# Ellon/pgslam

Hardware: AMD Instinct MI355X
Metric: ICP-converged scans/sec at 100k-pt scan vs 1M-pt local map (higher is better)
Workload: dtype f32; 1 GPU; scan-to-map ICP, 100000-pt Velodyne-shaped scan vs 1000000-pt local map, <=30 iterations (BASELINE.json configs[1]); distinct_scans=64, matcher=grid, streams=1, parallelism=1 independent replica(s), one process per GPU

## Files before the change

pgslam_amd/csrc/k_launch.inc:

```

static inline int cdiv(long long a, long long b) { return (int)((a + b - 1) / b); }
static inline int round8(int x) { return (x + 7) & ~7; }

template <typename T>
void launch_centroid_bbox_batch(hipStream_t st, const BuildDesc<T> *descs, int n, int max_m, unsigned long long *stats)
{
    int nb = cdiv(max_m, 256 * 8);
    if (nb < 1) nb = 1;
    if (nb > 512) nb = 512;
    hipLaunchKernelGGL(k_centroid_bbox_b<T>, dim3(nb, n), dim3(256), 0, st, descs, stats);
}

template <typename T>
void launch_grid_build_batch(hipStream_t st, const BuildDesc<T> *descs, int n, long long tot_m, long long tot_b, long long tot_s,
                             int max_m, int max_cells, int max_bins, int max_nsc, int max_blocks, int kx_all4, int *fkey, int *bins_a, int *block_sums,
                             int *cell_start, int *cell_start_f, int *bins_b, int *arrival, unsigned long long *words,
                             typename Vec4<T>::type *cpts, typename Vec4<T>::type *cnrm,
                             typename Vec4<T>::type *pts, typename Vec4<T>::type *nrm_out,
                             int *slot_of, int *sc_count, int *near, int *sc_dist, int *sc_wit, unsigned *occ, long long tot_o, float *sc_ext, float *ptsf,
                             uint4 *sw, int *ostart, int *flag_scratch, int *rank_scratch)
{
    (void)hipMemsetAsync(bins_a, 0, sizeof(int) * (tot_b + 1), st);
    (void)hipMemsetAsync(occ, 0, sizeof(unsigned) * tot_o, st);
    (void)hipMemsetAsync(sc_count, 0, sizeof(int) * tot_s, st);
// ... 87 lines not shown
}
constexpr int kTileGroupUnset = -0x7fffffff;
constexpr int kTileGroupDefault = 4;

template <typename T>
void launch_knn(hipStream_t st, int matcher, const ProblemDev *probs, const MapDev<T> *maps, const T *rd, int *slot,
                T *d2, const ChainDev<T> &ch, int P, int max_n, int use_seed, int *slow_count, int2 *slow_list, T *slow_lb,
                int *slow_ring, int fast_rings, const int *active, T *none_r, int n_problems, void *queue_buf, int clear_queue_counters,
                int table_kinds)
{
    if (matcher == 1) {
        (void)hipMemsetAsync(slow_count, 0, 4 * sizeof(int), st);
        hipLaunchKernelGGL(k_knn_brute<T>, dim3(cdiv(max_n, kKnnBlock), P), dim3(kKnnBlock), 0, st, probs, maps, rd, slot, d2,
                           ch, active);
        return;
    }
    const int nseg = n_problems * 8, q_cap = knn_q_cap(max_n);
    char *qb = (char *)queue_buf;
    int *seg_count = (int *)qb;                 qb += sizeof(int) * (size_t)nseg * kQueueCounterStride;
    int *seg_start = (int *)qb;                 qb += (sizeof(int) * (size_t)nseg + 255) & ~(size_t)255;
    int2 *seg_list = (int2 *)qb;                qb += sizeof(int2) * (size_t)nseg * q_cap;
    T *seg_lb = (T *)qb;                        qb += sizeof(T) * (size_t)nseg * q_cap;
    int *seg_ring = (int *)qb;
    if (clear_queue_counters) (void)hipMemsetAsync(seg_count, 0, sizeof(int) * (size_t)nseg * kQueueCounterStride, st);
    {
        static const int forced_lanes = env_knob("PGICP_FAST_LANES", 0);
        int lanes = kFastBlock;
        if ((long long)P * max_n >= 50000)
            while (lanes > 16 && (long long)P * cdiv(max_n, lanes >> 1) <= 8192) lanes >>= 1;
        if (forced_lanes > 0) lanes = std::min(forced_lanes, kFastBlock);
        static const int forced_group = env_knob("PGICP_TILE_GROUP", kTileGroupUnset);
        const int tile_group = forced_group != kTileGroupUnset ? forced_group : kTileGroupDefault;
        if (table_kinds & 1)
            hipLaunchKernelGGL((k_knn_grid<T, 1, 0>), dim3(round8(cdiv(max_n, lanes)), P), dim3(kFastBlock), 0, st, probs, maps, rd, slot, d2, ch,
                               use_seed, fast_rings, seg_count, seg_list, seg_lb, seg_ring, active, none_r, q_cap, lanes, tile_group);
        if (table_kinds & 2)
            hipLaunchKernelGGL((k_knn_grid<T, 1, 1>), dim3(round8(cdiv(max_n, lanes)), P), dim3(kFastBlock), 0, st, probs, maps, rd, slot, d2, ch,
                               use_seed, fast_rings, seg_count, seg_list, seg_lb, seg_ring, active, none_r, q_cap, lanes, tile_group);
    }
    if (P <= 8) {
        hipLaunchKernelGGL(k_queue_small<T>, dim3(P * 8, cdiv(q_cap, 256)), dim3(256), 0, st, (const int *)seg_count, nseg, q_cap,
                           (const int2 *)seg_list, (const T *)seg_lb, (const int *)seg_ring, slow_list, slow_lb, slow_ring, active, slow_count);
        return;
    }
    hipLaunchKernelGGL(k_queue_offsets, dim3(1), dim3(1024), 0, st, (const int *)seg_count, nseg, seg_start, slow_count);
    hipLaunchKernelGGL(k_queue_compact<T>, dim3(P * 8, cdiv(q_cap, 256)), dim3(256), 0, st, (const int *)seg_count, (const int *)seg_start,
                       q_cap, (const int2 *)seg_list, (const T *)seg_lb, (const int *)seg_ring, slow_list, slow_lb, slow_ring, active);
}

template <typename T>
void launch_borrow_order(hipStream_t st, const ProblemDev *probs, const SrcDesc *src, const int *order_a, const int *slot_a, const typename Vec4<T>::type *pts_a,
                         int first_a, int m_a, int n, const SeedSegs &sg, const int *slot_of_b, int m_b, T *rd_sorted, int *order_b, int *slot_b)
{
    hipLaunchKernelGGL(k_borrow_order<T>, dim3(cdiv(n, 256)), dim3(256), 0, st, probs, src, order_a, slot_a, pts_a, first_a, m_a, n, sg, slot_of_b, m_b, rd_sorted, order_b, slot_b);
}

template <typename T>
void launch_knn_med(hipStream_t st, ProblemDev *probs, const MapDev<T> *maps, const T *rd, int *slot, T *d2,
                    const ChainDev<T> &ch, int *slow_count, const int2 *slow_list, T *slow_lb, int *slow_ring, int *slow2_idx,
                    int med_rings, int use_seed, T *none_r)
{
    static const int short_rings = env_knob("PGICP_MED_SHORT_RINGS", 1);
    hipLaunchKernelGGL(k_knn_med<T>, dim3(8192), dim3(64), 0, st, probs, maps, rd, slot, d2, ch, slow_count, slow_list, slow_lb,
                       slow_ring, slow2_idx, med_rings, use_seed, none_r, short_rings);
}

template <typename T>
int launch_knn_topk(hipStream_t st, const ProblemDev *probs, const MapDev<T> *maps, const T *rd, int *slot, T *d2,
                    const ChainDev<T> &ch, int P, int max_n, const int *active)
{
    const dim3 grid(cdiv(max_n, 128), P), block(128);
// ... 337 lines not shown
```

pgslam_amd/csrc/k_match_common.inc:

```

template <typename T>
struct Best {
    T d2;
    int idx;
    int slot;
#ifdef PGICP_KNN_STATS
    int cnt = 0;
#endif
};

#ifdef PGICP_KNN_STATS
__device__ int g_trace_i = -1;
#define KNN_TRACE(prob_, i_, ...) do { if ((prob_) == 0 && (i_) == g_trace_i) printf(__VA_ARGS__); } while (0)
__device__ unsigned long long g_knn_stats[56];
__device__ unsigned *g_cnt_dump = nullptr;
__device__ float *g_d2_dump = nullptr;
__device__ long long g_dump_total = 0;
__device__ int g_dump_passes = 0;
#define KNN_STAT_WAVE_ADD(slot_, v_)                                                              \
    do {                                                                                          \
        long long s_ = (v_);                                                                      \
        for (int o_ = 32; o_ > 0; o_ >>= 1) s_ += __shfl_xor(s_, o_, 64);                          \
        if ((threadIdx.x & 63) == 0) atomicAdd(&g_knn_stats[slot_], (unsigned long long)s_);      \
    } while (0)
#define KNN_STAT_WAVE_MAX(slot_, v_)                                                              \
    do {                                                                                          \
        int s_ = (v_);                                                                            \
        for (int o_ = 32; o_ > 0; o_ >>= 1) s_ = max(s_, __shfl_xor(s_, o_, 64));                  \
        if ((threadIdx.x & 63) == 0) atomicAdd(&g_knn_stats[slot_], (unsigned long long)s_);      \
    } while (0)
#else
#define KNN_TRACE(prob_, i_, ...) do { } while (0)
#endif

#ifdef PGICP_PHASE_STATS
__device__ unsigned long long g_phase[64][3][16];
__device__ unsigned long long g_ball[16];
__device__ unsigned long long g_slow_worst[16];
#define PHASE_BEGIN() long long ph_t = (long long)__builtin_amdgcn_s_memtime(); unsigned ph_d[8] = {0, 0, 0, 0, 0, 0, 0, 0}
#define PHASE_MARK(k_) do { const long long t_ = (long long)__builtin_amdgcn_s_memtime(); ph_d[k_] += (unsigned)(t_ - ph_t); ph_t = t_; } while (0)
#define PHASE_FLUSH() do {                                                                                                  \
        if ((int)(threadIdx.x & 63) == __ffsll((long long)__ballot(1)) - 1) {                                              \
            unsigned long long *dst_ = g_phase[blockIdx.x & 63][use_seed ? 1 : 0];                                          \
            for (int k_ = 0; k_ < 8; ++k_) atomicAdd(dst_ + k_, (unsigned long long)ph_d[k_]);                              \
            atomicAdd(dst_ + 15, 1ULL);                                                                                     \
        } } while (0)
#define SPH_BEGIN() long long sph_t = (long long)__builtin_amdgcn_s_memtime(); const long long sph_t0 = sph_t; long long sph_e0 = sph_t; unsigned sph_emax = 0; unsigned sph_d[8] = {0, 0, 0, 0, 0, 0, 0, 0}; unsigned sph_n = 0
#define SPH_MARK(k_) do { const long long t_ = (long long)__builtin_amdgcn_s_memtime(); sph_d[k_] += (unsigned)(t_ - sph_t); sph_t = t_; } while (0)
#define SPH_ARRIVED(cond_) do { if (cond_) printf("x"); } while (0)
#define SPH_FLUSH() do {                                                                                                    \
        if ((threadIdx.x & 63) == 0) {                                                                                      \
            unsigned long long *dst_ = g_phase[blockIdx.x & 63][2];                                                         \
            for (int k_ = 0; k_ < 8; ++k_) atomicAdd(dst_ + k_, (unsigned long long)sph_d[k_]);                              \
            atomicAdd(dst_ + 14, (unsigned long long)sph_n); atomicAdd(dst_ + 15, 1ULL);                                    \
            atomicMax(dst_ + 12, (unsigned long long)(sph_t - sph_t0)); atomicMax(dst_ + 13, (unsigned long long)sph_emax);  \
        } } while (0)
#else
#define PHASE_BEGIN() do { } while (0)
#define PHASE_MARK(k_) do { } while (0)
#define PHASE_FLUSH() do { } while (0)
#define SPH_BEGIN() do { } while (0)
#define SPH_ARRIVED(cond_) do { } while (0)
#define SPH_MARK(k_) do { } while (0)
#define SPH_FLUSH() do { } while (0)
#endif

#ifdef PGICP_XCC_STATS
constexpr int kXccCopies = 32;
__device__ unsigned long long g_xcc[8][kXccCopies][16];
#define XCC_BEGIN() const unsigned long long xc_t0 = wall_clock64()
// ... 222 lines not shown
```

pgslam_amd/csrc/k_match_fast.inc:

```

template <typename T>
__device__ __forceinline__ T slab_far(T u, T lo, T hi)
{
    return fmax(fabs(u - lo), fabs(hi - u));
}

template <typename T>
__device__ __forceinline__ void finish_query(const MapDev<T> &M, const GridDesc<T> &g, const ChainDev<T> &ch, bool resolved, T gr,
                                             Best<T> best, T qx, T qy, T qz, T ux, T uy, T uz, int cx, int cy, int cz, int prob,
                                             int i, long long pos, int r_next, T lb_override, T free_r, int *__restrict__ slot_io,
                                             T *__restrict__ d2_out, T *__restrict__ none_r,
                                             int *__restrict__ slow_count, int2 *__restrict__ slow_list, T *__restrict__ slow_lb,
                                             int *__restrict__ slow_ring, int q_cap)
{
    if (resolved) {
        if (best.slot < 0) { best.d2 = Bits<T>::inf(); none_r[pos] = fmax(free_r, (T)0); }
        else none_r[pos] = sqrt(best.d2) * (T)0.9999;
    } else {
        T lb = lb_override >= (T)0 ? lb_override : (gr > (T)0 ? gr * gr : (T)0);
        if (free_r > (T)0) lb = fmax(lb, free_r * free_r);
        none_r[pos] = fmax(sqrt(lb) * (T)0.9999, free_r);
        if (best.slot < 0) {
            const int Cx = cx >> 3, Cy = cy >> 3, Cz = cz >> 3;
            const int wslot = as_global(M.sc_wit)[Cx + M.nsx * (Cy + M.nsy * Cz)];
// ... 45 lines not shown

template <typename T>
__global__ __launch_bounds__(256) void k_borrow_order(const ProblemDev *__restrict__ probs, const SrcDesc *__restrict__ src, const int *__restrict__ order_a,
                                                       const int *__restrict__ slot_a, const typename Vec4<T>::type *__restrict__ pts_a, int first_a, int m_a, int n, SeedSegs sg,
                                                       const int *__restrict__ slot_of_b, int m_b, T *__restrict__ rd_sorted, int *__restrict__ order_b,
                                                       int *__restrict__ slot_b)
{
    const int j = blockIdx.x * 256 + threadIdx.x;
    if (j >= n) return;
    const ProblemDev &P = probs[0];
    const SrcDesc sd = src[0];
    const int i = order_a[j];
    const T *in = (const T *)sd.ptr + (long long)i * sd.stride;
    T qx, qy, qz;
    apply_T<T>(P.Tpre, in[0], in[1], in[2], qx, qy, qz);
    T *dst = rd_sorted + 3 * (P.off + j);
    dst[0] = qx; dst[1] = qy; dst[2] = qz;
    order_b[P.off + j] = i;
    const int s = slot_a[j];
    int out = -1;
    if ((unsigned)s - (unsigned)first_a < (unsigned)m_a) {
        const int ia = Bits<T>::unpack_idx(pts_a[s].w);
        for (int k = 0; k < sg.n; ++k)
            if (ia >= sg.src[k] && ia < sg.src[k + 1]) {
                const unsigned off = (unsigned)ia - (unsigned)sg.src[k];
                if (sg.dst[k] >= 0 && sg.dst[k] < m_b && off < (unsigned)(m_b - sg.dst[k])) out = slot_of_b[sg.dst[k] + (int)off];
                break;
            }
    }
    slot_b[P.off + j] = out;
}
constexpr int kFastBlock = PGICP_FAST_BLOCK;

template <typename T, int R, int TK>
__global__ __launch_bounds__(kFastBlock) PGICP_FAST_ATTR void k_knn_grid(const ProblemDev *__restrict__ probs, const MapDev<T> *__restrict__ maps,
                                                  const T *__restrict__ rd, int *__restrict__ slot_io,
                                                  T *__restrict__ d2_out, ChainDev<T> ch, int use_seed, int fast_rings,
                                                  int *__restrict__ slow_count, int2 *__restrict__ slow_list,
                                                  T *__restrict__ slow_lb, int *__restrict__ slow_ring,
                                                  const int *__restrict__ active, T *__restrict__ none_r, int q_cap, int lanes, int tile_group)
{
    using V4 = typename Vec4<T>::type;
    constexpr int NR = (2 * R + 1) * (2 * R + 1);
    constexpr bool kItems = kFastBlock == 64;
    constexpr bool kBallPool = kItems && PGICP_RING_POOL;
    __shared__ __attribute__((aligned(16))) int lds_raw[2 * kItemsMax + (sizeof(T) == 4 ? 6 : 12) * kFastBlock];
    static_assert(sizeof(lds_raw) >= sizeof(int) * 2 * (NR - 1) * kFastBlock && kItemsMax >= (NR - 1) * kFastBlock, "the list view and one item per range must fit");
    int (*rng_a)[kFastBlock] = reinterpret_cast<int (*)[kFastBlock]>(lds_raw);
    int (*rng_b)[kFastBlock] = reinterpret_cast<int (*)[kFastBlock]>(lds_raw + (NR - 1) * kFastBlock);
    const int prob = active[blockIdx.y];
    const ProblemDev &P = probs[prob];
    if (P.done) return;
    const int tile = tile_of_block(blockIdx.x, gridDim.x, tile_group);
    const int lane = threadIdx.x;
    const int i = tile * lanes + lane;
    if (tile * lanes >= P.n) return;
    PHASE_BEGIN();
    XCC_BEGIN();
    bool live = lane < lanes && i < P.n;
    const MapDev<T> M = maps[P.map];
    if ((M.sw != nullptr) != (TK == 1)) return;
    const GridDesc<T> g = M.g;
    T qx = 0, qy = 0, qz = 0;
    const T cap2 = (use_seed & 1) ? (T)(1.21 * P.rlimit) : Bits<T>::inf();
    const bool capped = cap2 < ch.max_dist2;
    bool still_none = false, skip = false;
    T free_r = (T)0;
    Best<T> best, seed;
    best.d2 = capped ? cap2 : ch.max_dist2;
    best.idx = 0x7FFFFFFF;
    best.slot = -1;
    seed.d2 = Bits<T>::inf(); seed.idx = 0x7FFFFFFF; seed.slot = -1;
    int dsc = 0;
    if (live) {
        const T *q = rd + 3 * (P.off + i);
        apply_T<T>(tcur_of<T>(P), q[0], q[1], q[2], qx, qy, qz);
        {
            const int sx = clamp_cell<T>(qx - g.ox, g.inv_h, g.nx) >> 3, sy8 = clamp_cell<T>(qy - g.oy, g.inv_h, g.ny) >> 3,
                      sz8 = clamp_cell<T>(qz - g.oz, g.inv_h, g.nz) >> 3;
// ... 149 lines not shown
#pragma unroll
            for (int u = 0; u < NP; ++u) { c0[u] = load_rec<T>(M.pts, pv[u] ? pj[u] : 0); c1[u] = load_rec<T>(M.pts, pt[u] ? pj[u] + 1 : 0); }
#pragma unroll
            for (int u = 0; u < NP; ++u) {
                eval_point_if<T>(pv[u], c0[u], pj[u], qx, qy, qz, best);
                eval_point_if<T>(pt[u], c1[u], pj[u] + 1, qx, qy, qz, best);
            }
#ifdef PGICP_KNN_STATS
            flat_iters += 2;
#endif
        }
    }
    }
    }
#ifdef PGICP_KNN_STATS
    KNN_STAT_WAVE_MAX(3, flat_iters);
    KNN_STAT_WAVE_ADD(4, best.cnt - cnt_a1);
    if (live) {
        atomicAdd(&g_knn_stats[16 + (cnt_a1 <= 0 ? 0 : min(15, 32 - __clz(cnt_a1)))], 1ULL);
        const int c2 = best.cnt - cnt_a1;
        atomicAdd(&g_knn_stats[32 + (c2 <= 0 ? 0 : min(15, 32 - __clz(c2)))], 1ULL);
    }
    const int cnt_a = best.cnt;
    const bool dump_on = g_cnt_dump && P.iters < g_dump_passes && lane < lanes && i < P.n;
    if (dump_on) {
        g_cnt_dump[(long long)P.iters * g_dump_total + P.off + i] = (unsigned)min(cnt_a1, 1023) | ((unsigned)min(cnt_a - cnt_a1, 1023) << 10);
        g_d2_dump[(long long)P.iters * g_dump_total + P.off + i] = use_seed ? (float)seed.d2 : -1.0f;
    }
#endif
    PHASE_MARK(4);
    if (!__any(live)) { PHASE_FLUSH(); XCC_END(); }
    if constexpr (!kBallPool) { if (!live) return; }

    T gr;
    int r_next;
    bool resolved;
    if constexpr (kBallPool) {
        if constexpr (sizeof(T) == 4)
            resolved = grid_nn_ball<T, TK>(M, lane, search, qx, qy, qz, ch.max_dist, R, fast_rings, cap2, best, gr, r_next, items, sq, skey, nullptr, sslot, pool_n);
        else {
            T *sqd = reinterpret_cast<T *>(lds_raw + 2 * kItemsMax);
            unsigned long long *skd = reinterpret_cast<unsigned long long *>(lds_raw + 2 * kItemsMax + 6 * kFastBlock);
            int *sxd = lds_raw + 2 * kItemsMax + 8 * kFastBlock, *ssd = lds_raw + 2 * kItemsMax + 9 * kFastBlock;
            unsigned *fbd = reinterpret_cast<unsigned *>(lds_raw + 2 * kItemsMax + 10 * kFastBlock);
            float *sud = reinterpret_cast<float *>(lds_raw + 2 * kItemsMax + 11 * kFastBlock);
            resolved = grid_nn_ball<T, TK>(M, lane, search, qx, qy, qz, ch.max_dist, R, fast_rings, cap2, best, gr, r_next, items, sqd, skd, sxd, ssd, pool_n, fbd, sud);
        }
        if (!live) return;
    } else {
        resolved = false; gr = (T)0; r_next = R + 1;
        if (search) resolved = grid_nn<T>(M, qx, qy, qz, ch.max_dist, R + 1, fast_rings, cap2, best, gr, r_next);
    }
    PHASE_MARK(5);
#ifdef PGICP_KNN_STATS
    atomicAdd(&g_knn_stats[5], (unsigned long long)(best.cnt - cnt_a));
    atomicAdd(&g_knn_stats[6], (unsigned long long)(resolved ? 0 : 1));
    atomicAdd(&g_knn_stats[7], (unsigned long long)(best.cnt > cnt_a ? 1 : 0));
    KNN_STAT_WAVE_MAX(8, best.cnt - cnt_a);
    KNN_STAT_WAVE_MAX(9, best.cnt);
    if (dump_on) g_cnt_dump[(long long)P.iters * g_dump_total + P.off + i] |= (unsigned)min(best.cnt - cnt_a, 4095) << 20;
#endif
    KNN_TRACE(prob, i, "[fast] i=%d use_seed=%d capped=%d cap2=%g best=(%g,%d) seed=(%g,%d) resolved=%d gr=%g r_next=%d\n", i, use_seed, (int)capped, (double)cap2, (double)best.d2, best.slot, (double)seed.d2, seed.slot, (int)resolved, (double)gr, r_next);
    T lb_override = (T)-1;
    if (skip) {
        resolved = false;
        r_next = 0;
        gr = (T)0;
    }
    if (capped && best.slot < 0) {
        if (resolved) lb_override = cap2;
        resolved = false;
        if (seed.slot >= 0 && seed.d2 <= ch.max_dist2) best = seed;
// ... 9 lines not shown
```

pgslam_amd/csrc/k_match_pool.inc:

```
#ifndef PGICP_ITEMS_MAX
#define PGICP_ITEMS_MAX 512
#endif
#ifndef PGICP_ITEM_CHUNK
#define PGICP_ITEM_CHUNK 8
#endif
constexpr int kItemsMax = PGICP_ITEMS_MAX;
#ifndef PGICP_ITEM_CHUNK_F
#define PGICP_ITEM_CHUNK_F 4
#endif
#ifndef PGICP_ITEM_CHUNK_D
#define PGICP_ITEM_CHUNK_D PGICP_ITEM_CHUNK
#endif
template <typename T> struct ItemChunk { static constexpr int n = sizeof(T) == 4 ? PGICP_ITEM_CHUNK_F : PGICP_ITEM_CHUNK_D;
                                         static constexpr int shift = n == 4 ? 2 : n == 8 ? 3 : n == 16 ? 4 : n == 32 ? 5 : -1; };
constexpr int kItemShift = ItemChunk<float>::shift;
static_assert(ItemChunk<float>::shift > 0 && ItemChunk<double>::shift > 0, "the item size is a power of two (items are counted with shifts: a division by a run-time size costs ~30 VALU instructions)");

__device__ __forceinline__ void item_rounds(const float4 *__restrict__ pts, const int2 *items, int total, const float *sq,
                                            unsigned long long *skey, int *sslot, int lane, int chunk)
{
    __syncthreads();
    for (int b0 = 0; b0 < total; b0 += 64) {
        const int it = b0 + lane;
        const int2 I = it < total ? items[it] : make_int2(0, 0);
// ... 226 lines not shown
    }
    if (total == 0) return;
    const int chunk = 1 << sh;
    int w = incl - mine;
#pragma unroll
    for (int t = 0; t < N; ++t) {
        const int len = rb[t] - ra[t];
        if (len > 0) { items[w] = make_int2(ra[t], (min(len, chunk) << 6) | lane); ++w; }
        if (__any(len > chunk)) {
#pragma clang loop vectorize(disable) unroll(disable)
            for (int a = ra[t] + chunk; a < rb[t]; a += chunk) { items[w] = make_int2(a, (min(rb[t] - a, chunk) << 6) | lane); ++w; }
        }
    }
    const unsigned long long key0 = (unsigned long long)__double_as_longlong(best.d2);
    const int idx0 = best.idx;
    sq[lane] = qx; sq[64 + lane] = qy; sq[128 + lane] = qz;
    skey[lane] = key0;
    sidx[lane] = idx0;
    sslot[lane] = best.slot;
    if (ptsf) { fb[lane] = __float_as_uint(bk_up(best.d2)); item_rounds_dp(pts, ptsf, items, total, sq, skey, sidx, sslot, fb, su, lane, chunk); }
    else item_rounds_d(pts, items, total, sq, skey, sidx, sslot, lane, chunk);
    const unsigned long long kf = skey[lane];
    const int xf = sidx[lane];
    if (kf != key0 || xf != idx0) { best.d2 = __longlong_as_double((long long)kf); best.idx = xf; best.slot = sslot[lane]; }
}

#ifndef PGICP_RING_POOL
#define PGICP_RING_POOL 1
#endif
#ifndef PGICP_FREE_SKIP
#define PGICP_FREE_SKIP 1
#endif
constexpr int kPoolCap = kItemsMax - 1;
#ifndef PGICP_BALL_ROWS
#define PGICP_BALL_ROWS 2
#endif
constexpr int kBallRows = PGICP_BALL_ROWS;
constexpr int kPoolFlushAt = kPoolCap - 128 * kBallRows;
template <typename T, int TK = 2>
__device__ __forceinline__ bool grid_nn_ball(const MapDev<T> &M, int lane, bool active, T qx, T qy, T qz, T max_dist,
                                             int r_done, int max_rings, T stop_d2, Best<T> &best, T &gr_out, int &r_next,
                                             int2 *items, T *sq, unsigned long long *skey, int *sidx, int *sslot, int *pool_n,
                                             unsigned *fb = nullptr, const float *su = nullptr)
{
    r_next = r_done + 1;
    const GridDesc<T> g = M.g;
    const int c0x = clamp_cell<T>(qx - g.ox, g.inv_h, g.nx), c0y = clamp_cell<T>(qy - g.oy, g.inv_h, g.ny), c0z = clamp_cell<T>(qz - g.oz, g.inv_h, g.nz);
    GridDesc<BK> gb;
    gb.h = (BK)g.h; gb.inv_h = (BK)g.inv_h; gb.margin = bk_margin<T>(g, qx - g.ox, qy - g.oy, qz - g.oz); gb.nx = g.nx; gb.ny = g.ny; gb.nz = g.nz;
    const BK ux = (BK)(qx - g.ox), uy = (BK)(qy - g.oy), uz = (BK)(qz - g.oz);
    const BK bmax = (BK)max_dist, bstop = (BK)stop_d2;
    BK bbest = bk_up(best.d2);
    gr_out = (T)0;
    bool resolved = false, open = active;
    if (open) {
        BK gr = ring_guarantee<BK>(gb, ux, uy, uz, c0x, c0y, c0z, r_done);
        if (!(gr < Bits<BK>::inf())) { resolved = true; open = false; }
        else {
            gr = gr - gb.margin;
            gr_out = (T)gr;
            if (gr > (BK)0 && (bbest < gr * gr || gr > bmax)) { resolved = true; open = false; }
            else if (gr > (BK)0 && gr * gr > bstop) open = false;
        }
    }
    if (max_rings <= r_done || !__any(open)) return resolved;
    const typename Vec4<T>::type *pts = M.pts;
    const int kx = M.kx, nxf = g.nx * kx;
    const BK inv_hx = gb.inv_h * (BK)kx;
    const int sy = __builtin_amdgcn_readfirstlane(nxf), sz = __builtin_amdgcn_readfirstlane(nxf * g.ny);
    sq[lane] = qx; sq[64 + lane] = qy; sq[128 + lane] = qz;
    if constexpr (sizeof(T) == 4) skey[lane] = item_key(best.d2, best.idx);
    else { skey[lane] = (unsigned long long)__double_as_longlong(best.d2); sidx[lane] = best.idx; if (fb) fb[lane] = __float_as_uint(bk_up(best.d2)); }
    sslot[lane] = best.slot;
    if (lane == 0) *pool_n = 0;
    __syncthreads();
#ifdef PGICP_PHASE_STATS
    int st_trips = 0, st_items = 0, st_flush = 0;
#endif
    auto push = [&](int a, int b) {
        constexpr int kItemChunk = ItemChunk<T>::n;
        const int n = (b - a + kItemChunk - 1) >> ItemChunk<T>::shift;
        const int w = atomicAdd(pool_n, n);
        if (w + n <= kPoolCap) {
            items[w] = make_int2(a, (min(b - a, kItemChunk) << 6) | lane);
#pragma clang loop vectorize(disable) unroll(disable)
            for (int k = 1; k < n; ++k) items[w + k] = make_int2(a + k * kItemChunk, (min(b - a - k * kItemChunk, kItemChunk) << 6) | lane);
        } else {
#pragma clang loop vectorize(disable) unroll(disable)
            for (int k = w; k < kPoolCap; ++k) items[k] = make_int2(0, lane);
            scan_range<T>(pts, a, b, qx, qy, qz, best);
        }
    };
    auto flush = [&]() {
        __syncthreads();
        const int total = min(__builtin_amdgcn_readfirstlane(*pool_n), kPoolCap);
        if (total > 0) {
#ifdef PGICP_PHASE_STATS
            st_items += total; ++st_flush;
#endif
            if constexpr (sizeof(T) == 4) {
                item_rounds(pts, items, total, sq, skey, sslot, lane, ItemChunk<T>::n);
                const unsigned long long kf = skey[lane];
                if (kf < item_key(best.d2, best.idx)) { best.d2 = __uint_as_float((unsigned)(kf >> 32)); best.idx = (int)(unsigned)kf; best.slot = sslot[lane]; }
            } else {
                if (fb && M.ptsf) item_rounds_dp(pts, reinterpret_cast<const float4 *>(M.ptsf), items, total, sq, skey, sidx, sslot, fb, su, lane, ItemChunk<T>::n);
                else item_rounds_d(pts, items, total, sq, skey, sidx, sslot, lane, ItemChunk<T>::n);
                const unsigned long long kf = skey[lane], kb = (unsigned long long)__double_as_longlong(best.d2);
                const int xf = sidx[lane];
                if (kf < kb || (kf == kb && xf < best.idx)) { best.d2 = __longlong_as_double((long long)kf); best.idx = xf; best.slot = sslot[lane]; }
                skey[lane] = (unsigned long long)__double_as_longlong(best.d2); sidx[lane] = best.idx; sslot[lane] = best.slot;
                if (fb) fb[lane] = __float_as_uint(bk_up(best.d2));
            }
            bbest = bk_up(best.d2);
            if (lane == 0) *pool_n = 0;
            __syncthreads();
        }
    };
    const BK rho = bk_sqrt(bbest) * (BK)1.000001 + gb.margin;
    const int ylo = max(c0y - max_rings, clamp_cell<BK>(uy - rho, gb.inv_h, g.ny)), yhi = min(c0y + max_rings, clamp_cell<BK>(uy + rho, gb.inv_h, g.ny));
    const int zlo = max(c0z - max_rings, clamp_cell<BK>(uz - rho, gb.inv_h, g.nz)), zhi = min(c0z + max_rings, clamp_cell<BK>(uz + rho, gb.inv_h, g.nz));
    const BK wl_all = (BK)(max(c0x - max_rings, 0) * kx), wh_all = (BK)(min(c0x + max_rings, g.nx - 1) * kx + kx - 1);
    const BK wh_left = (BK)((c0x - r_done) * kx - 1), wl_right = (BK)((c0x + r_done) * kx + kx);
#ifdef PGICP_PHASE_STATS
    const int st_open = __popcll(__ballot(open));
    int st_rows = open ? (yhi - ylo + 1) * (zhi - zlo + 1) : 0;
    for (int o_ = 32; o_ > 0; o_ >>= 1) st_rows += __shfl_xor(st_rows, o_, 64);
#endif
    int y = ylo, z = zlo;
    int rowb = nxf * (ylo + g.ny * zlo);
    const int wrap = sz - (yhi - ylo + 1) * sy;
    bool walking = open;
#if PGICP_BALL_ROWS > 1
    while (__any(walking)) {
        constexpr int NW = 2 * kBallRows;
        int ia[NW], ib[NW];
        bool need[NW];
#pragma unroll
        for (int w = 0; w < NW; ++w) { ia[w] = 0; ib[w] = 0; need[w] = false; }
#pragma unroll
        for (int r = 0; r < kBallRows; ++r) {
            if (walking) {
                const BK ly = fmax(slab_dist<BK>(uy, y, gb.h) - gb.margin, (BK)0), lz = fmax(slab_dist<BK>(uz, z, gb.h) - gb.margin, (BK)0);
                const BK lb2 = ly * ly + lz * lz;
                if (!(lb2 > bbest)) {
                    const BK rad = bk_sqrt(fmax(bbest - lb2, (BK)0)) * (BK)1.000001 + gb.margin;
                    const BK flo = floor((ux - rad) * inv_hx), fhi = floor((ux + rad) * inv_hx);
                    const bool inside = abs(y - c0y) <= r_done && abs(z - c0z) <= r_done;
#pragma unroll
                    for (int k = 0; k < 2; ++k) {
                        const BK wl = (inside && k == 1) ? wl_right : wl_all, wh = (inside && k == 0) ? wh_left : wh_all;
                        const bool on = (k == 0 || inside) && !(wl > wh || fhi < wl || flo > wh);
                        need[2 * r + k] = on;
                        ia[2 * r + k] = rowb + (int)fmax(flo, wl); ib[2 * r + k] = rowb + (int)fmin(fhi, wh) + 1;
                    }
                }
                ++y; rowb += sy;
                if (y > yhi) { y = ylo; ++z; rowb += wrap; walking = z <= zhi; }
            }
        }
        int va[NW], vb[NW];
#pragma unroll
        for (int w = 0; w < NW; ++w) { va[w] = 0; vb[w] = 0; if (need[w]) tab_range_k<TK, T>(M, ia[w], ib[w], va[w], vb[w]); }
#pragma unroll
        for (int w = 0; w < NW; ++w) if (va[w] < vb[w]) push(va[w], vb[w]);
#ifdef PGICP_PHASE_STATS
        ++st_trips;
#endif
        __syncthreads();
        if (__builtin_amdgcn_readfirstlane(*pool_n) >= kPoolFlushAt) flush();
    }
#else
    while (__any(walking)) {
        if (walking) {
            const BK ly = fmax(slab_dist<BK>(uy, y, gb.h) - gb.margin, (BK)0), lz = fmax(slab_dist<BK>(uz, z, gb.h) - gb.margin, (BK)0);
            const BK lb2 = ly * ly + lz * lz;
            if (!(lb2 > bbest)) {
                const BK rad = bk_sqrt(fmax(bbest - lb2, (BK)0)) * (BK)1.000001 + gb.margin;
                const BK flo = floor((ux - rad) * inv_hx), fhi = floor((ux + rad) * inv_hx);
                const bool inside = abs(y - c0y) <= r_done && abs(z - c0z) <= r_done;
#pragma unroll 1
                for (int k = 0; k < (inside ? 2 : 1); ++k) {
                    const BK wl = (inside && k == 1) ? wl_right : wl_all, wh = (inside && k == 0) ? wh_left : wh_all;
                    if (wl > wh || fhi < wl || flo > wh) continue;
                    const int fa = (int)fmax(flo, wl), fb = (int)fmin(fhi, wh);
                    int a, b;
                    tab_range_k<TK, T>(M, rowb + fa, rowb + fb + 1, a, b);
                    if (a < b) push(a, b);
                }
            }
            ++y; rowb += sy;
            if (y > yhi) { y = ylo; ++z; rowb += wrap; walking = z <= zhi; }
        }
#ifdef PGICP_PHASE_STATS
        ++st_trips;
#endif
        __syncthreads();
        if (__builtin_amdgcn_readfirstlane(*pool_n) >= kPoolFlushAt) flush();
    }
#endif
    flush();
#ifdef PGICP_PHASE_STATS
    if (lane == 0) {
        atomicAdd(&g_ball[0], 1ULL); atomicAdd(&g_ball[1], (unsigned long long)st_open); atomicAdd(&g_ball[2], (unsigned long long)st_trips);
        atomicAdd(&g_ball[4], (unsigned long long)st_items); atomicAdd(&g_ball[5], (unsigned long long)st_flush);
        atomicAdd(&g_ball[7], (unsigned long long)st_rows);
    }
#endif
    if (open) {
        BK gr = ring_guarantee<BK>(gb, ux, uy, uz, c0x, c0y, c0z, max_rings);
        if (!(gr < Bits<BK>::inf())) resolved = true;
        else {
            gr = gr - gb.margin;
            gr_out = (T)gr;
            bbest = bk_up(best.d2);
            if (gr > (BK)0 && (bbest < gr * gr || gr > bmax)) resolved = true;
            else r_next = max_rings + 1;
        }
    }
    return resolved;
}
```

pgslam_amd/csrc/k_minimise.inc:

```

__device__ __forceinline__ void accumulate_pair(double *acc, double w, double px, double py, double pz, double qx,
                                                double qy, double qz, double nx, double ny, double nz)
{
    const double dx = px - qx, dy = py - qy, dz = pz - qz;
    const double e = (nx * dx + ny * dy) + nz * dz;
    double J[6];
    J[0] = py * nz - pz * ny;
    J[1] = pz * nx - px * nz;
    J[2] = px * ny - py * nx;
    J[3] = nx; J[4] = ny; J[5] = nz;
    int k = 0;
#pragma unroll
    for (int a = 0; a < 6; a++)
#pragma unroll
        for (int b = a; b < 6; b++) acc[k++] += w * (J[a] * J[b]);
#pragma unroll
    for (int a = 0; a < 6; a++) acc[21 + a] -= w * (J[a] * e);
    acc[27] += w;
    acc[28] += 1.0;
    acc[29] += w * (e * e);
}

constexpr int kDppShl4 = 0x104, kDppShr4 = 0x114, kDppRor8 = 0x128, kDppQuadXor2 = 0x4E, kDppQuadXor1 = 0xB1;

// ... 438 lines not shown

__global__ __launch_bounds__(256) void k_reopen(ProblemDev *__restrict__ probs, int P)
{
    const int p = blockIdx.x * blockDim.x + threadIdx.x;
    if (p < P && probs[p].status == PGICP_ST_OK) probs[p].done = 0;
}
void launch_reopen(hipStream_t st, ProblemDev *probs, int P)
{
    hipLaunchKernelGGL(k_reopen, dim3((P + 255) / 256), dim3(256), 0, st, probs, P);
}

int knn_trace_set(int sorted_index)
{
#ifdef PGICP_KNN_STATS
    return hipMemcpyToSymbol(HIP_SYMBOL(g_trace_i), &sorted_index, sizeof(int)) == hipSuccess ? 0 : -1;
#else
    (void)sorted_index;
    return -1;
#endif
}

int knn_phase_read(unsigned long long out[48], int reset)
{
#ifdef PGICP_PHASE_STATS
    static unsigned long long h[64 * 48];
    if (hipMemcpyFromSymbol(h, HIP_SYMBOL(g_phase), sizeof h) != hipSuccess) return -1;
    for (int k = 0; k < 48; k++) {
        out[k] = 0;
        const bool is_max = k == 32 + 12 || k == 32 + 13;
        for (int c = 0; c < 64; c++) out[k] = is_max ? std::max(out[k], h[c * 48 + k]) : out[k] + h[c * 48 + k];
    }
    if (reset) { std::memset(h, 0, sizeof h); (void)hipMemcpyToSymbol(HIP_SYMBOL(g_phase), h, sizeof h); }
    {
        unsigned long long b[16];
        if (hipMemcpyFromSymbol(b, HIP_SYMBOL(g_ball), sizeof b) == hipSuccess && b[0])
            std::fprintf(stderr, "      ball walk: %llu waves; per wave: %.1f open lanes, %.1f trips, %.1f items in %.2f evaluations; %.1f rows per open lane\n",
                         b[0], (double)b[1] / b[0], (double)b[2] / b[0], (double)b[4] / b[0], (double)b[5] / b[0], b[1] ? (double)b[7] / b[1] : 0.0);
        if (reset) { std::memset(b, 0, sizeof b); (void)hipMemcpyToSymbol(HIP_SYMBOL(g_ball), b, sizeof b); }
    }
    {
        unsigned long long w[16];
        if (hipMemcpyFromSymbol(w, HIP_SYMBOL(g_slow_worst), sizeof w) == hipSuccess && w[0])
            std::fprintf(stderr, "      slowest entry: %llu cycles [fetch %llu seed %llu look-ups %llu points %llu walk %llu finish %llu]; square of %llu rows, %llu with points, %llu long, %llu candidates; bounded %llu capped %llu, result at %llu mm\n",
                         w[0], w[1], w[2], w[3], w[4], w[5], w[6], w[8], w[9], w[10], w[11], w[12], w[13], w[14]);
        if (reset) { std::memset(w, 0, sizeof w); (void)hipMemcpyToSymbol(HIP_SYMBOL(g_slow_worst), w, sizeof w); }
    }
    return 0;
#else
    (void)out; (void)reset;
    return -1;
#endif
}

int knn_xcc_report(int use_seed, int reset)
{
#ifdef PGICP_XCC_STATS
    static unsigned long long h[8][kXccCopies][16];
    if (hipMemcpyFromSymbol(h, HIP_SYMBOL(g_xcc), sizeof h) != hipSuccess) return -1;
    unsigned long long x[8][16] = {};
    for (int c = 0; c < 8; c++)
        for (int k = 0; k < kXccCopies; k++)
            for (int s = 0; s < 16; s++) x[c][s] = s < 2 ? std::max(x[c][s], h[c][k][s]) : x[c][s] + h[c][k][s];
    unsigned long long first = ~0ULL;
    for (int c = 0; c < 8; c++) if (x[c][3]) first = std::min(first, ~x[c][0]);
    std::fprintf(stderr, "    fast kernel per XCC (seeded %d) [last end after the launch's first start | wave time summed | waves | waves by blockIdx.x & 7], ticks of 10 ns:", use_seed);
    for (int c = 0; c < 8; c++) {
        std::fprintf(stderr, " %llu|%llu|%llu|", x[c][3] ? x[c][1] - first : 0ULL, x[c][2], x[c][3]);
        for (int k = 0; k < 8; k++) std::fprintf(stderr, "%s%llu", k ? "," : "", x[c][8 + k]);
    }
    std::fprintf(stderr, "\n");
// ... 288 lines not shown
```

pgslam_amd/csrc/kernels.hip:

```cpp
#include "kernels.hpp"
#include "tile_map.hpp"
#include <algorithm>
#include <cstdio>
#include <cstdlib>
#include <cstring>
#include <limits>
#include <map>
#include <type_traits>
#ifndef PGICP_FAST_BLOCK
#define PGICP_FAST_BLOCK 64
#endif
#ifndef PGICP_FAST_WAVES
#define PGICP_FAST_WAVES 6
#endif
#ifndef PGICP_FAST_ATTR
#ifndef PGICP_FAST_WAVES_D
#define PGICP_FAST_WAVES_D 4
#endif
#define PGICP_FAST_ATTR __attribute__((amdgpu_num_sgpr(80), amdgpu_waves_per_eu(sizeof(T) == 4 ? PGICP_FAST_WAVES : PGICP_FAST_WAVES_D, sizeof(T) == 4 ? PGICP_FAST_WAVES : PGICP_FAST_WAVES_D)))
#endif

namespace pgicp {

template <typename T> struct Bits;
template <> struct Bits<float> {
    using U = unsigned int;
    static constexpr int kBits = 32;
    __device__ static U key(float v) { return __float_as_uint(v); }
    __device__ static float val(U k) { return __uint_as_float(k); }
    __device__ static float pack_idx(int i) { return __int_as_float(i); }
    __device__ static int unpack_idx(float w) { return __float_as_int(w); }
    __device__ static float inf() { return __uint_as_float(0x7F800000u); }
};
template <> struct Bits<double> {
// ... 138 lines not shown
```

Baseline: 13030 scans/s.

## Deal ball-walk row chunks across wave lanes to balance imbalanced per-lane boxes

Adds a load-balanced mode to the grid ball search. When per-lane row counts are skewed enough, the rows of every lane's yz box are dealt evenly across all 64 lanes through LDS, so each lane scans another lane's rows and pushes items tagged with the owner. It also adds a template flag so the kNN kernel skips the ring-walk path when fast_rings is 1. The dealt mode adds LDS space, extra barriers and per-owner reads from shared memory in exchange for fewer idle lanes in imbalanced waves.

New measurement: 13200 scans/s, median of 6. 1.01x the previous value.

```diff
diff --git a/pgslam_amd/csrc/ball_rows.hpp b/pgslam_amd/csrc/ball_rows.hpp
--- /dev/null
+++ b/pgslam_amd/csrc/ball_rows.hpp
@@ -0,0 +1,35 @@
+#pragma once
+
+#if defined(__HIPCC__) || defined(__CUDACC__)
+#define PGICP_BALL_HD __host__ __device__ __forceinline__
+#else
+#define PGICP_BALL_HD inline
+#endif
+
+namespace pgicp {
+
+constexpr int kBallDealMaxRings = 7;
+
+PGICP_BALL_HD unsigned ball_box_pack(int ny, int nz, int dylo, int dzlo)
+{
+    return ((unsigned)ny << 12) | ((unsigned)nz << 8) | ((unsigned)dylo << 4) | (unsigned)dzlo;
+}
+PGICP_BALL_HD int ball_box_ny(unsigned w) { return (int)((w >> 12) & 15u); }
+PGICP_BALL_HD int ball_box_nz(unsigned w) { return (int)((w >> 8) & 15u); }
+PGICP_BALL_HD int ball_box_dylo(unsigned w) { return (int)((w >> 4) & 15u); }
+PGICP_BALL_HD int ball_box_dzlo(unsigned w) { return (int)(w & 15u); }
+
+PGICP_BALL_HD int ball_chunks(int n, int per) { return (n + per - 1) / per; }
+
+PGICP_BALL_HD void ball_row_yz(int r, int ny, float inv_ny, int &dy, int &dz)
+{
+    dz = (int)(((float)r + 0.5f) * inv_ny);
+    dy = r - dz * ny;
+}
+
+PGICP_BALL_HD int ball_deal_place(int first, int below, int window) { return first - window + below; }
+PGICP_BALL_HD unsigned ball_deal_word(int k, int lane) { return ((unsigned)k << 6) | (unsigned)lane; }
+PGICP_BALL_HD int ball_deal_owner(unsigned w) { return (int)(w & 63u); }
+PGICP_BALL_HD int ball_deal_chunk(unsigned w) { return (int)(w >> 6); }
+
+}
diff --git a/pgslam_amd/csrc/k_launch.inc b/pgslam_amd/csrc/k_launch.inc
--- a/pgslam_amd/csrc/k_launch.inc
+++ b/pgslam_amd/csrc/k_launch.inc
@@ -143,11 +143,11 @@
         static const int forced_group = env_knob("PGICP_TILE_GROUP", kTileGroupUnset);
         const int tile_group = forced_group != kTileGroupUnset ? forced_group : kTileGroupDefault;
         if (table_kinds & 1)
-            hipLaunchKernelGGL((k_knn_grid<T, 1, 0>), dim3(round8(cdiv(max_n, lanes)), P), dim3(kFastBlock), 0, st, probs, maps, rd, slot, d2, ch,
-                               use_seed, fast_rings, seg_count, seg_list, seg_lb, seg_ring, active, none_r, q_cap, lanes, tile_group);
+            hipLaunchKernelGGL((fast_rings > 1 ? k_knn_grid<T, 1, 0, true> : k_knn_grid<T, 1, 0, false>), dim3(round8(cdiv(max_n, lanes)), P), dim3(kFastBlock), 0, st,
+                               probs, maps, rd, slot, d2, ch, use_seed, fast_rings, seg_count, seg_list, seg_lb, seg_ring, active, none_r, q_cap, lanes, tile_group);
         if (table_kinds & 2)
-            hipLaunchKernelGGL((k_knn_grid<T, 1, 1>), dim3(round8(cdiv(max_n, lanes)), P), dim3(kFastBlock), 0, st, probs, maps, rd, slot, d2, ch,
-                               use_seed, fast_rings, seg_count, seg_list, seg_lb, seg_ring, active, none_r, q_cap, lanes, tile_group);
+            hipLaunchKernelGGL((fast_rings > 1 ? k_knn_grid<T, 1, 1, true> : k_knn_grid<T, 1, 1, false>), dim3(round8(cdiv(max_n, lanes)), P), dim3(kFastBlock), 0, st,
+                               probs, maps, rd, slot, d2, ch, use_seed, fast_rings, seg_count, seg_list, seg_lb, seg_ring, active, none_r, q_cap, lanes, tile_group);
     }
     if (P <= 8) {
         hipLaunchKernelGGL(k_queue_small<T>, dim3(P * 8, cdiv(q_cap, 256)), dim3(256), 0, st, (const int *)seg_count, nseg, q_cap,
diff --git a/pgslam_amd/csrc/k_match_common.inc b/pgslam_amd/csrc/k_match_common.inc
--- a/pgslam_amd/csrc/k_match_common.inc
+++ b/pgslam_amd/csrc/k_match_common.inc
@@ -35,7 +35,7 @@
 
 #ifdef PGICP_PHASE_STATS
 __device__ unsigned long long g_phase[64][3][16];
-__device__ unsigned long long g_ball[16];
+__device__ unsigned long long g_ball[2][16];
 __device__ unsigned long long g_slow_worst[16];
 #define PHASE_BEGIN() long long ph_t = (long long)__builtin_amdgcn_s_memtime(); unsigned ph_d[8] = {0, 0, 0, 0, 0, 0, 0, 0}
 #define PHASE_MARK(k_) do { const long long t_ = (long long)__builtin_amdgcn_s_memtime(); ph_d[k_] += (unsigned)(t_ - ph_t); ph_t = t_; } while (0)
diff --git a/pgslam_amd/csrc/k_match_fast.inc b/pgslam_amd/csrc/k_match_fast.inc
--- a/pgslam_amd/csrc/k_match_fast.inc
+++ b/pgslam_amd/csrc/k_match_fast.inc
@@ -101,7 +101,7 @@
 }
 constexpr int kFastBlock = PGICP_FAST_BLOCK;
 
-template <typename T, int R, int TK>
+template <typename T, int R, int TK, bool WALK = true>
 __global__ __launch_bounds__(kFastBlock) PGICP_FAST_ATTR void k_knn_grid(const ProblemDev *__restrict__ probs, const MapDev<T> *__restrict__ maps,
                                                   const T *__restrict__ rd, int *__restrict__ slot_io,
                                                   T *__restrict__ d2_out, ChainDev<T> ch, int use_seed, int fast_rings,
@@ -113,7 +113,7 @@
     constexpr int NR = (2 * R + 1) * (2 * R + 1);
     constexpr bool kItems = kFastBlock == 64;
     constexpr bool kBallPool = kItems && PGICP_RING_POOL;
-    __shared__ __attribute__((aligned(16))) int lds_raw[2 * kItemsMax + (sizeof(T) == 4 ? 6 : 12) * kFastBlock];
+    __shared__ __attribute__((aligned(16))) int lds_raw[2 * kItemsMax + (sizeof(T) == 4 ? 6 + 3 * PGICP_BALL_DEAL : 12) * kFastBlock];
     static_assert(sizeof(lds_raw) >= sizeof(int) * 2 * (NR - 1) * kFastBlock && kItemsMax >= (NR - 1) * kFastBlock, "the list view and one item per range must fit");
     int (*rng_a)[kFastBlock] = reinterpret_cast<int (*)[kFastBlock]>(lds_raw);
     int (*rng_b)[kFastBlock] = reinterpret_cast<int (*)[kFastBlock]>(lds_raw + (NR - 1) * kFastBlock);
@@ -329,12 +329,14 @@
     if (!__any(live)) { PHASE_FLUSH(); XCC_END(); }
     if constexpr (!kBallPool) { if (!live) return; }
 
+    if constexpr (!WALK) fast_rings = R;
     T gr;
     int r_next;
     bool resolved;
     if constexpr (kBallPool) {
         if constexpr (sizeof(T) == 4)
-            resolved = grid_nn_ball<T, TK>(M, lane, search, qx, qy, qz, ch.max_dist, R, fast_rings, cap2, best, gr, r_next, items, sq, skey, nullptr, sslot, pool_n);
+            resolved = grid_nn_ball<T, TK>(M, lane, search, qx, qy, qz, ch.max_dist, R, fast_rings, cap2, best, gr, r_next, items, sq, skey, nullptr, sslot, pool_n, nullptr, nullptr,
+                                            reinterpret_cast<unsigned *>(lds_raw + 2 * kItemsMax + 6 * kFastBlock));
         else {
             T *sqd = reinterpret_cast<T *>(lds_raw + 2 * kItemsMax);
             unsigned long long *skd = reinterpret_cast<unsigned long long *>(lds_raw + 2 * kItemsMax + 6 * kFastBlock);
diff --git a/pgslam_amd/csrc/k_match_pool.inc b/pgslam_amd/csrc/k_match_pool.inc
--- a/pgslam_amd/csrc/k_match_pool.inc
+++ b/pgslam_amd/csrc/k_match_pool.inc
@@ -282,6 +282,12 @@
 #define PGICP_FREE_SKIP 1
 #endif
 constexpr int kPoolCap = kItemsMax - 1;
+#ifndef PGICP_BALL_DEAL
+#define PGICP_BALL_DEAL 1
+#endif
+#ifndef PGICP_BALL_DEAL_GAIN
+#define PGICP_BALL_DEAL_GAIN 65
+#endif
 #ifndef PGICP_BALL_ROWS
 #define PGICP_BALL_ROWS 2
 #endif
@@ -291,7 +297,7 @@
 __device__ __forceinline__ bool grid_nn_ball(const MapDev<T> &M, int lane, bool active, T qx, T qy, T qz, T max_dist,
                                              int r_done, int max_rings, T stop_d2, Best<T> &best, T &gr_out, int &r_next,
                                              int2 *items, T *sq, unsigned long long *skey, int *sidx, int *sslot, int *pool_n,
-                                             unsigned *fb = nullptr, const float *su = nullptr)
+                                             unsigned *fb = nullptr, const float *su = nullptr, [[maybe_unused]] unsigned *sown = nullptr)
 {
     r_next = r_done + 1;
     const GridDesc<T> g = M.g;
@@ -325,7 +331,7 @@
     if (lane == 0) *pool_n = 0;
     __syncthreads();
 #ifdef PGICP_PHASE_STATS
-    int st_trips = 0, st_items = 0, st_flush = 0;
+    int st_trips = 0, st_items = 0, st_flush = 0, st_kept = 0;
 #endif
     auto push = [&](int a, int b) {
         constexpr int kItemChunk = ItemChunk<T>::n;
@@ -380,6 +386,135 @@
     int rowb = nxf * (ylo + g.ny * zlo);
     const int wrap = sz - (yhi - ylo + 1) * sy;
     bool walking = open;
+#if PGICP_BALL_DEAL
+    if constexpr (sizeof(T) == 4) {
+        if (max_rings <= kBallDealMaxRings) {
+            const int nyb = yhi - ylo + 1, nzb = zhi - zlo + 1;
+            const int mine = open ? ball_chunks(nyb * nzb, kBallRows) : 0;
+            int total = mine, most = mine;
+#pragma unroll
+            for (int o = 32; o > 0; o >>= 1) { total += __shfl_xor(total, o, 64); most = max(most, __shfl_xor(most, o, 64)); }
+            if (100 * ((total + 63) >> 6) <= PGICP_BALL_DEAL_GAIN * most) {
+                walking = false;
+                unsigned *sfc = sown + 64;
+                sown[lane] = open ? ball_box_pack(nyb, nzb, c0y - ylo, c0z - zlo) : 0u;
+                sfc[lane] = (unsigned)(c0x * kx);
+                unsigned *shead = sown + 128;
+                int lev = 0, lev0 = 0;
+                __syncthreads();
+                const unsigned *skey_hi = reinterpret_cast<const unsigned *>(skey) + 1;
+                auto flush_dealt = [&]() {
+                    __syncthreads();
+                    const int n_items = min(__builtin_amdgcn_readfirstlane(*pool_n), kPoolCap);
+                    if (n_items > 0) {
+#ifdef PGICP_PHASE_STATS
+                        st_items += n_items; ++st_flush;
+#endif
+                        item_rounds(pts, items, n_items, sq, skey, sslot, lane, ItemChunk<T>::n);
+                        if (lane == 0) *pool_n = 0;
+                        __syncthreads();
+                    }
+                };
+                for (int cb = 0; cb < total; cb += 64) {
+                    const bool valid = cb + lane < total;
+                    for (int k = lev, first = lev0; first < cb + 64 && k < most; ++k) {
+                        const unsigned long long in = __ballot(mine > k);
+                        const int pos = ball_deal_place(first, (int)__builtin_amdgcn_mbcnt_hi((unsigned)(in >> 32), __builtin_amdgcn_mbcnt_lo((unsigned)in, 0u)), cb);
+                        if (mine > k && pos >= 0 && pos < 64) shead[pos] = ball_deal_word(k, lane);
+                        first += __popcll(in);
+                        if (first <= cb + 64) { lev = k + 1; lev0 = first; }
+                    }
+                    __syncthreads();
+                    const unsigned hv = shead[lane];
+                    const int owner = ball_deal_owner(hv), lchunk = valid ? ball_deal_chunk(hv) : 0x7FFF;
+                    const unsigned bw = sown[owner];
+                    const int ony = ball_box_ny(bw), orows = ony * ball_box_nz(bw);
+                    const BK oux = sq[owner] - g.ox, ouy = sq[64 + owner] - g.oy, ouz = sq[128 + owner] - g.oz;
+                    const int ocy = clamp_cell<T>(ouy, g.inv_h, g.ny), ocz = clamp_cell<T>(ouz, g.inv_h, g.nz);
+                    const int fc = (int)sfc[owner];
+                    const BK owl_all = (BK)max(fc - max_rings * kx, 0), owh_all = (BK)min(fc + max_rings * kx + kx - 1, nxf - 1);
+                    const BK owh_left = (BK)(fc - r_done * kx - 1), owl_right = (BK)(fc + r_done * kx + kx);
+                    int r = lchunk * kBallRows, dy, dz;
+                    ball_row_yz(r, ony, __builtin_amdgcn_rcpf((float)ony), dy, dz);
+                    const int oylo = ocy - ball_box_dylo(bw);
+                    int yy = oylo + dy, zz = ocz - ball_box_dzlo(bw) + dz;
+                    int orow = nxf * (yy + g.ny * zz);
+                    bool going = valid && r < orows;
+                    const BK obest = __uint_as_float(skey_hi[2 * owner]);
+                    constexpr int NW = 2 * kBallRows;
+                    int ia[NW], ib[NW];
+                    bool need[NW];
+#pragma unroll
+                    for (int w = 0; w < NW; ++w) { ia[w] = 0; ib[w] = 0; need[w] = false; }
+#pragma unroll
+                    for (int k = 0; k < kBallRows; ++k) {
+                        if (going) {
+                            const BK ly = fmax(slab_dist<BK>(ouy, yy, gb.h) - gb.margin, (BK)0), lz = fmax(slab_dist<BK>(ouz, zz, gb.h) - gb.margin, (BK)0);
+                            const BK lb2 = ly * ly + lz * lz;
+                            if (!(lb2 > obest)) {
+#ifdef PGICP_PHASE_STATS
+                                ++st_kept;
+#endif
+                                const BK rad = bk_sqrt(fmax(obest - lb2, (BK)0)) * (BK)1.000001 + gb.margin;
+                                const BK flo = floor((oux - rad) * inv_hx), fhi = floor((oux + rad) * inv_hx);
+                                const bool inside = abs(yy - ocy) <= r_done && abs(zz - ocz) <= r_done;
+#pragma unroll
+                                for (int e = 0; e < 2; ++e) {
+                                    const BK wl = (inside && e == 1) ? owl_right : owl_all, wh = (inside && e == 0) ? owh_left : owh_all;
+                                    const bool on = (e == 0 || inside) && !(wl > wh || fhi < wl || flo > wh);
+                                    need[2 * k + e] = on;
+                                    ia[2 * k + e] = orow + (int)fmax(flo, wl); ib[2 * k + e] = orow + (int)fmin(fhi, wh) + 1;
+                                }
+                            }
+                            ++yy; orow += sy; ++r;
+                            if (yy >= oylo + ony) { yy = oylo; ++zz; orow += sz - ony * sy; }
+                            going = r < orows;
+                        }
+                    }
+                    int va[NW], vb[NW];
+#pragma unroll
+                    for (int w = 0; w < NW; ++w) { va[w] = 0; vb[w] = 0; if (need[w]) tab_range_k<TK, T>(M, ia[w], ib[w], va[w], vb[w]); }
+                    Best<T> ov;
+                    ov.d2 = Bits<T>::inf(); ov.idx = 0x7FFFFFFF; ov.slot = -1;
+#pragma unroll
+                    for (int w = 0; w < NW; ++w) if (va[w] < vb[w]) {
+                        constexpr int kItemChunk = ItemChunk<T>::n;
+                        const int a = va[w], b = vb[w], n = (b - a + kItemChunk - 1) >> ItemChunk<T>::shift;
+                        const int at = atomicAdd(pool_n, n);
+                        if (at + n <= kPoolCap) {
+                            items[at] = make_int2(a, (min(b - a, kItemChunk) << 6) | owner);
+#pragma clang loop vectorize(disable) unroll(disable)
+                            for (int k = 1; k < n; ++k) items[at + k] = make_int2(a + k * kItemChunk, (min(b - a - k * kItemChunk, kItemChunk) << 6) | owner);
+                        } else {
+#pragma clang loop vectorize(disable) unroll(disable)
+                            for (int k = at; k < kPoolCap; ++k) items[k] = make_int2(0, owner);
+                            scan_range<T>(pts, a, b, sq[owner], sq[64 + owner], sq[128 + owner], ov);
+                        }
+                    }
+#ifdef PGICP_PHASE_STATS
+                    ++st_trips;
+#endif
+                    if (__any(ov.slot >= 0)) {
+                        const unsigned long long key = item_key(ov.d2, ov.idx);
+                        const bool cand = ov.slot >= 0 && key < skey[owner];
+                        if (cand) atomicMin(&skey[owner], key);
+                        __syncthreads();
+                        if (cand && skey[owner] == key) sslot[owner] = ov.slot;
+                    }
+                    __syncthreads();
+                    if (__builtin_amdgcn_readfirstlane(*pool_n) >= kPoolFlushAt) flush_dealt();
+                }
+                flush_dealt();
+                const unsigned long long kf = skey[lane];
+                best.d2 = __uint_as_float((unsigned)(kf >> 32)); best.idx = (int)(unsigned)kf; best.slot = sslot[lane];
+                bbest = bk_up(best.d2);
+#ifdef PGICP_PHASE_STATS
+                if (lane == 0) atomicAdd(&g_ball[stop_d2 < Bits<T>::inf() ? 1 : 0][6], 1ULL);
+#endif
+            }
+        }
+    }
+#endif
 #if PGICP_BALL_ROWS > 1
     while (__any(walking)) {
         constexpr int NW = 2 * kBallRows;
@@ -393,6 +528,9 @@
                 const BK ly = fmax(slab_dist<BK>(uy, y, gb.h) - gb.margin, (BK)0), lz = fmax(slab_dist<BK>(uz, z, gb.h) - gb.margin, (BK)0);
                 const BK lb2 = ly * ly + lz * lz;
                 if (!(lb2 > bbest)) {
+#ifdef PGICP_PHASE_STATS
+                    ++st_kept;
+#endif
                     const BK rad = bk_sqrt(fmax(bbest - lb2, (BK)0)) * (BK)1.000001 + gb.margin;
                     const BK flo = floor((ux - rad) * inv_hx), fhi = floor((ux + rad) * inv_hx);
                     const bool inside = abs(y - c0y) <= r_done && abs(z - c0z) <= r_done;
@@ -425,6 +563,9 @@
             const BK ly = fmax(slab_dist<BK>(uy, y, gb.h) - gb.margin, (BK)0), lz = fmax(slab_dist<BK>(uz, z, gb.h) - gb.margin, (BK)0);
             const BK lb2 = ly * ly + lz * lz;
             if (!(lb2 > bbest)) {
+#ifdef PGICP_PHASE_STATS
+                ++st_kept;
+#endif
                 const BK rad = bk_sqrt(fmax(bbest - lb2, (BK)0)) * (BK)1.000001 + gb.margin;
                 const BK flo = floor((ux - rad) * inv_hx), fhi = floor((ux + rad) * inv_hx);
                 const bool inside = abs(y - c0y) <= r_done && abs(z - c0z) <= r_done;
@@ -450,10 +591,13 @@
 #endif
     flush();
 #ifdef PGICP_PHASE_STATS
+    for (int o_ = 32; o_ > 0; o_ >>= 1) st_kept += __shfl_xor(st_kept, o_, 64);
     if (lane == 0) {
-        atomicAdd(&g_ball[0], 1ULL); atomicAdd(&g_ball[1], (unsigned long long)st_open); atomicAdd(&g_ball[2], (unsigned long long)st_trips);
-        atomicAdd(&g_ball[4], (unsigned long long)st_items); atomicAdd(&g_ball[5], (unsigned long long)st_flush);
-        atomicAdd(&g_ball[7], (unsigned long long)st_rows);
+        unsigned long long *gb_ = g_ball[stop_d2 < Bits<T>::inf() ? 1 : 0];
+        atomicAdd(&gb_[0], 1ULL); atomicAdd(&gb_[1], (unsigned long long)st_open); atomicAdd(&gb_[2], (unsigned long long)st_trips);
+        atomicAdd(&gb_[3], (unsigned long long)st_kept);
+        atomicAdd(&gb_[4], (unsigned long long)st_items); atomicAdd(&gb_[5], (unsigned long long)st_flush);
+        atomicAdd(&gb_[7], (unsigned long long)st_rows);
     }
 #endif
     if (open) {
diff --git a/pgslam_amd/csrc/k_minimise.inc b/pgslam_amd/csrc/k_minimise.inc
--- a/pgslam_amd/csrc/k_minimise.inc
+++ b/pgslam_amd/csrc/k_minimise.inc
@@ -494,10 +494,14 @@
     }
     if (reset) { std::memset(h, 0, sizeof h); (void)hipMemcpyToSymbol(HIP_SYMBOL(g_phase), h, sizeof h); }
     {
-        unsigned long long b[16];
-        if (hipMemcpyFromSymbol(b, HIP_SYMBOL(g_ball), sizeof b) == hipSuccess && b[0])
-            std::fprintf(stderr, "      ball walk: %llu waves; per wave: %.1f open lanes, %.1f trips, %.1f items in %.2f evaluations; %.1f rows per open lane\n",
-                         b[0], (double)b[1] / b[0], (double)b[2] / b[0], (double)b[4] / b[0], (double)b[5] / b[0], b[1] ? (double)b[7] / b[1] : 0.0);
+        unsigned long long b[2][16];
+        if (hipMemcpyFromSymbol(b, HIP_SYMBOL(g_ball), sizeof b) == hipSuccess)
+            for (int u = 0; u < 2; u++)
+                if (b[u][0])
+                    std::fprintf(stderr, "      ball walk, %s: %llu waves (%llu dealt); per wave: %.1f open lanes, %.1f trips, %.1f box rows, %.1f rows kept, %.1f items in %.2f evaluations; %.1f box rows per open lane; row-slot utilisation %.3f (box rows %.3f)\n",
+                                 u ? "seeded passes" : "unseeded pass", b[u][0], b[u][6], (double)b[u][1] / b[u][0], (double)b[u][2] / b[u][0], (double)b[u][7] / b[u][0], (double)b[u][3] / b[u][0],
+                                 (double)b[u][4] / b[u][0], (double)b[u][5] / b[u][0], b[u][1] ? (double)b[u][7] / b[u][1] : 0.0,
+                                 b[u][2] ? (double)b[u][3] / (64.0 * kBallRows * b[u][2]) : 0.0, b[u][2] ? (double)b[u][7] / (64.0 * kBallRows * b[u][2]) : 0.0);
         if (reset) { std::memset(b, 0, sizeof b); (void)hipMemcpyToSymbol(HIP_SYMBOL(g_ball), b, sizeof b); }
     }
     {
diff --git a/pgslam_amd/csrc/kernels.hip b/pgslam_amd/csrc/kernels.hip
--- a/pgslam_amd/csrc/kernels.hip
+++ b/pgslam_amd/csrc/kernels.hip
@@ -1,5 +1,6 @@
 #include "kernels.hpp"
 #include "tile_map.hpp"
+#include "ball_rows.hpp"
 #include <algorithm>
 #include <cstdio>
 #include <cstdlib>
```
